# gongweibao/FleetX

Hardware: AMD Instinct MI355X
Metric: tokens/sec (whole node) GPT-3 6.7B hybrid-parallel at 1/2/4/8 MI355X (higher is better)
Workload: dtype bf16; 1 GPU; model=gpt3-6.7B, global_batch=8, seq_len=1024, parallelism=dp1, micro_batch=8, hip_graph=True, grad_reduce_dtype=float32, recompute=False

## Files before the change

### csrc/kernels/bindings.cpp

```cpp
#include <hip/hip_runtime.h>
#include <pybind11/pybind11.h>
#include <pybind11/stl.h>
#include <stdint.h>
#include <string>
#include <stdexcept>
#include <vector>

namespace py = pybind11;
typedef uintptr_t ptr;

#include "fx_api.h"

#define P(x) reinterpret_cast<void*>(x)
#define CP(x) reinterpret_cast<const void*>(x)
#define S(x) reinterpret_cast<hipStream_t>(x)
#define F(x) reinterpret_cast<float*>(x)

static std::vector<long> v3(const std::vector<long>& a) {
  std::vector<long> r(a);
  r.resize(3, 0);
  return r;
}

PYBIND11_MODULE(_kernels, m) {
  m.doc() = "FleetX-AMD HIP kernels (gfx950)";
  m.def("coltile_splits", &fx_coltile_splits);
  m.def("add_ln_fwd", [](int dt, ptr x, ptr bias, ptr res, ptr g, ptr b, ptr s_out, ptr y,
                         ptr mean, ptr rstd, int rows, int h, float eps, float p, uint64_t key,
                         ptr salt, ptr st) {
    fx_add_ln_fwd(dt, CP(x), CP(bias), CP(res), CP(g), CP(b), P(s_out), P(y), F(mean), F(rstd),
                  rows, h, eps, p, key, CP(salt), S(st));
  });
  m.def("ln_bwd_row", [](int dt, ptr dy, ptr s, ptr mean, ptr rstd, ptr g, ptr ds_in, ptr ds_out,
                         ptr dx_out, int rows, int h, float p, uint64_t key, ptr salt, ptr st) {
    fx_ln_bwd_row(dt, CP(dy), CP(s), F(mean), F(rstd), CP(g), CP(ds_in), P(ds_out), P(dx_out),
                  rows, h, p, key, CP(salt), S(st));
  });
  m.def("ln_bwd_cols_blocks", &fx_ln_bwd_cols_blocks);
  m.def("ln_bwd_cols", [](int dt, ptr dy, ptr s, ptr mean, ptr rstd, ptr g, ptr ds_in, ptr ds_out,
                          ptr dx_out, int rows, int h, float p, uint64_t key, ptr part,
                          int with_dbias, ptr fg, ptr tg, int accg, ptr fb, ptr tb, int accb,
                          ptr fx, ptr tx, int accx, ptr salt, ptr st) {
    return fx_ln_bwd_cols(dt, CP(dy), CP(s), F(mean), F(rstd), CP(g), CP(ds_in), P(ds_out),
                          P(dx_out), rows, h, p, key, F(part), with_dbias, F(fg), P(tg), accg,
                          F(fb), P(tb), accb, F(fx), P(tx), accx, CP(salt), S(st));
  }, py::arg("dt"), py::arg("dy"), py::arg("s"), py::arg("mean"), py::arg("rstd"), py::arg("g"),
     py::arg("ds_in"), py::arg("ds_out"), py::arg("dx_out"), py::arg("rows"), py::arg("h"),
     py::arg("p"), py::arg("key"), py::arg("part"), py::arg("with_dbias"), py::arg("fg") = 0,
     py::arg("tg") = 0, py::arg("accg") = 0, py::arg("fb") = 0, py::arg("tb") = 0,
     py::arg("accb") = 0, py::arg("fx") = 0, py::arg("tx") = 0, py::arg("accx") = 0,
     py::arg("salt") = 0, py::arg("st") = 0);
  m.def("coltile_partial", [](int dt, int mode, ptr a, ptr b, ptr mean, ptr rstd, ptr p0, ptr p1,
                              int rows, int cols, int splits, ptr st, ptr cnt, ptr f0, ptr t0,
                              int acc0, ptr f1, ptr t1, int acc1) {
    fx_coltile_partial(dt, mode, CP(a), CP(b), F(mean), F(rstd), F(p0), F(p1), rows, cols, splits,
                       S(st), reinterpret_cast<int*>(cnt), F(f0), P(t0), acc0, F(f1), P(t1),
                       acc1);
  }, py::arg("dt"), py::arg("mode"), py::arg("a"), py::arg("b"), py::arg("mean"), py::arg("rstd"),
     py::arg("p0"), py::arg("p1"), py::arg("rows"), py::arg("cols"), py::arg("splits"),
     py::arg("st"), py::arg("cnt") = 0, py::arg("f0") = 0, py::arg("t0") = 0, py::arg("acc0") = 0,
     py::arg("f1") = 0, py::arg("t1") = 0, py::arg("acc1") = 0);
  m.def("coltile_finalize", [](int dt, ptr part, int splits, int cols, ptr out_f32, ptr out_t,
                               int accumulate, ptr st) {
    fx_coltile_finalize(dt, F(part), splits, cols, F(out_f32), P(out_t), accumulate, S(st));
  });
  m.def("bias_gelu_fwd", [](int dt, int erf, ptr x, ptr bias, ptr y, long n, int cols, ptr st) {
    fx_bias_gelu_fwd(dt, erf, CP(x), CP(bias), P(y), n, cols, S(st));
  });
  m.def("bias_gelu_bwd", [](int dt, int erf, ptr dy, ptr x, ptr bias, ptr dx, ptr part, int rows,
                            int cols, int splits, ptr st, ptr cnt, ptr out_f32, ptr out_t,
                            int acc) {
    fx_bias_gelu_bwd(dt, erf, CP(dy), CP(x), CP(bias), P(dx), F(part), rows, cols, splits, S(st),
                     reinterpret_cast<int*>(cnt), F(out_f32), P(out_t), acc);
  }, py::arg("dt"), py::arg("erf"), py::arg("dy"), py::arg("x"), py::arg("bias"), py::arg("dx"),
     py::arg("part"), py::arg("rows"), py::arg("cols"), py::arg("splits"), py::arg("st"),
     py::arg("cnt") = 0, py::arg("out_f32") = 0, py::arg("out_t") = 0, py::arg("acc") = 0);
  m.def("bias_dropout_add_fwd", [](int dt, ptr x, ptr bias, ptr res, ptr out, long n, int cols,
                                   float p, uint64_t key, ptr salt, ptr st) {
    fx_bias_dropout_add_fwd(dt, CP(x), CP(bias), CP(res), P(out), n, cols, p, key, CP(salt),
                            S(st));
  });
  m.def("dropout_bwd_colsum", [](int dt, ptr dout, ptr dx, ptr part, int rows, int cols,
                                 int splits, float p, uint64_t key, ptr salt, ptr st, ptr cnt,
                                 ptr out_f32, ptr out_t, int acc) {
    fx_dropout_bwd_colsum(dt, CP(dout), P(dx), F(part), rows, cols, splits, p, key, CP(salt), S(st),
                          reinterpret_cast<int*>(cnt), F(out_f32), P(out_t), acc);
  }, py::arg("dt"), py::arg("dout"), py::arg("dx"), py::arg("part"), py::arg("rows"),
     py::arg("cols"), py::arg("splits"), py::arg("p"), py::arg("key"), py::arg("salt"),
     py::arg("st"), py::arg("cnt") = 0, py::arg("out_f32") = 0, py::arg("out_t") = 0,
     py::arg("acc") = 0);
  m.def("dropout_fwd", [](int dt, ptr x, ptr y, long n, float p, uint64_t key, ptr salt,
                          ptr st) {
    fx_dropout_fwd(dt, CP(x), P(y), n, p, key, CP(salt), S(st));
  });
  m.def("ce_stats", [](int dt, ptr logits, ptr labels, int rows, int V, long vstart, ptr mx,
                       ptr sm, ptr tg, int ignore, ptr st) {
    fx_ce_stats(dt, CP(logits), reinterpret_cast<const int64_t*>(labels), rows, V, vstart, F(mx),
                F(sm), F(tg), ignore, S(st));
  });
  m.def("ce_bwd", [](int dt, ptr logits, ptr dx, ptr labels, ptr lse, ptr g, int rows, int V,
                     long vstart, int ignore, ptr st) {
    fx_ce_bwd(dt, CP(logits), P(dx), reinterpret_cast<const int64_t*>(labels), F(lse), F(g), rows,
              V, vstart, ignore, S(st));
  });
  m.def("sumsq_blocks", &fx_sumsq_blocks);
  m.def("sumsq_chunks", [](ptr addr, ptr len, int n, ptr partial, ptr st) {
    fx_sumsq_chunks(reinterpret_cast<const int64_t*>(addr), reinterpret_cast<const int64_t*>(len),
                    n, F(partial), S(st));
  });
  m.def("sumsq_f32", [](ptr x, long n, ptr partial, int blocks, ptr st) {
    fx_sumsq_f32(F(x), n, F(partial), blocks, S(st));
  });
  m.def("sumsq_16", [](int dt, ptr x, long n, ptr partial, int blocks, ptr st) {
    fx_sumsq_16(dt, CP(x), n, F(partial), blocks, S(st));
  });
  m.def("adamw", [](int dt, int flags, ptr p, ptr g, ptr mm, ptr vv, ptr p16, long n, float lr,
                    float b1, float b2, float eps, float wd, float l2, ptr gscale, ptr skip,
                    ptr step, ptr lr_dev, int grid, int nt, int wide, ptr st) {
    return fx_adamw(dt, flags, P(p), CP(g), F(mm), F(vv), P(p16), n, lr, b1, b2, eps, wd, l2,
                    F(gscale), reinterpret_cast<const int*>(skip),
                    reinterpret_cast<const int*>(step), F(lr_dev), grid, nt, wide, S(st));
  });
  m.def("pk_split", [](ptr x, ptr hi, ptr lo, long n, ptr st) {
    fx_pk_split(F(x), P(hi), P(lo), n, S(st));
  });
  m.def("pk_join", [](ptr hi, ptr lo, ptr x, long n, ptr st) {
// ... 177 lines not shown
```

### csrc/kernels/fx_api.h

```cpp
#pragma once
#include <hip/hip_runtime.h>
#include <stdint.h>

extern "C" {
int fx_coltile_splits(int rows, int cols);
void fx_add_ln_fwd(int, const void*, const void*, const void*, const void*, const void*, void*,
                   void*, float*, float*, int, int, float, float, uint64_t, const void*,
                   hipStream_t);
void fx_ln_bwd_row(int, const void*, const void*, const float*, const float*, const void*,
                   const void*, void*, void*, int, int, float, uint64_t, const void*, hipStream_t);
int fx_ln_bwd_cols_blocks(int, int, int);
int fx_ln_bwd_cols(int, const void*, const void*, const float*, const float*, const void*,
                   const void*, void*, void*, int, int, float, uint64_t, float*, int, float*, void*,
                   int, float*, void*, int, float*, void*, int, const void*, hipStream_t);
void fx_coltile_partial(int, int, const void*, const void*, const float*, const float*, float*,
                        float*, int, int, int, hipStream_t, int*, float*, void*, int, float*,
                        void*, int);
void fx_coltile_finalize(int, const float*, int, int, float*, void*, int, hipStream_t);
void fx_bias_gelu_fwd(int, int, const void*, const void*, void*, long, int, hipStream_t);
void fx_bias_gelu_bwd(int, int, const void*, const void*, const void*, void*, float*, int, int, int,
                      hipStream_t, int*, float*, void*, int);
void fx_bias_dropout_add_fwd(int, const void*, const void*, const void*, void*, long, int, float,
                             uint64_t, const void*, hipStream_t);
void fx_dropout_bwd_colsum(int, const void*, void*, float*, int, int, int, float, uint64_t,
                           const void*, hipStream_t, int*, float*, void*, int);
void fx_dropout_fwd(int, const void*, void*, long, float, uint64_t, const void*, hipStream_t);
void fx_ce_stats(int, const void*, const int64_t*, int, int, long, float*, float*, float*, int,
                 hipStream_t);
void fx_ce_bwd(int, const void*, void*, const int64_t*, const float*, const float*, int, int, long,
               int, hipStream_t);
int fx_sumsq_blocks(long n);
void fx_sumsq_f32(const float*, long, float*, int, hipStream_t);
void fx_sumsq_16(int, const void*, long, float*, int, hipStream_t);
void fx_sumsq_chunks(const int64_t*, const int64_t*, int, float*, hipStream_t);
int fx_adamw(int dtype, int flags, void* master, const void* grad, float* m, float* v, void* p16,
             long n, float lr, float beta1, float beta2, float eps, float wd, float l2,
             const float* gscale, const int* skip, const int* step, const float* lr_dev,
             int grid_cap, int nt, int wide, hipStream_t st);
void fx_pk_split(const float*, void*, void*, long, hipStream_t);
void fx_pk_join(const void*, const void*, float*, long, hipStream_t);
void fx_cast_f32(int, const float*, void*, long, hipStream_t);
void fx_accum_f32(int, float*, const void*, long, int, hipStream_t);
void fx_embedding_fwd(int, const int64_t*, const int64_t*, const void*, const void*, void*, int,
                      int, long, long, hipStream_t);
void fx_embedding_bwd(int, const int64_t*, const void*, float*, int, int, long, long,
                      hipStream_t);
void fx_fa_set_dkdv64(int);
void fx_fa_set_dq64(int);
void fx_fa_set_dkdv_vreg(int);
int fx_fa_lab();
int fx_fa_set_stamps(void*);
int fx_flash_fwd(int, const void*, const void*, const void*, void*, float*, const long*, const long*,
                 const long*, const long*, const int*, const float*, long, int, int, int, int, int,
                 int, float, float, uint64_t, const void*, hipStream_t);
int fx_flash_bwd(int, const void*, const void*, const void*, const void*, const void*, const float*,
                 float*, void*, void*, void*, const long*, const long*, const long*, const long*,
                 const long*, const long*, const int*, const float*, long, int, int, int, int, int,
                 int, float, float, uint64_t, const void*, hipStream_t);
int fx_fake_quant_fwd(int, const void*, void*, const float*, int, long, hipStream_t);
void fx_absmax(int, const void*, long, float*, hipStream_t);
int fx_gn_nseg(long, long);
int fx_gn_fwd(int, const void*, const float*, const float*, const float*, const float*, void*,
              double*, float*, float*, int, int, int, long, int, float, int, hipStream_t);
int fx_gn_bwd_reduce(int, const void*, const void*, const float*, const float*, const float*,
                     const float*, const float*, const float*, float*, int, int, int, long, int,
                     int, hipStream_t);
int fx_gn_bwd_apply(int, const void*, const void*, const float*, const float*, const float*,
                    const float*, const float*, const float*, const float*, const float*, void*,
                    int, int, int, long, int, int, hipStream_t);
int fx_transpose16(int, const void*, void*, float*, int, int, long, long, hipStream_t);
int fx_sample(int, const void*, long, int, int, float, int, float, const float*, int64_t*, float*,
              float*, hipStream_t);
int fx_decode_attn(int, const void*, const void*, const void*, void*, const int*, int, int, int,
                   int, int, float*, long, long, long, long, long, long, float, hipStream_t);
int fx_beam_decode_attn(int, const void*, const void*, const void*, const int*, const void*,
                        const void*, const int*, const int*, void*, float*, int, int, int, int, int,
                        int, int, long, long, long, long, long, long, long, long, long, long, float,
                        int, hipStream_t);
void fx_embedding_bwd_sorted(int, const int64_t*, const int64_t*, const void*, float*, int, int,
                             long, long, hipStream_t);
int fx_softmax_fwd(int, int, const void*, const void*, void*, long, int, int, long, float, int,
                   hipStream_t);
int fx_softmax_bwd(int, const void*, const void*, void*, long, int, int, float, int, hipStream_t);
int fx_gemm(int, int, int, int, int, int, int, const void*, long, const void*, long, void*, long,
            const void*, void*, long, int, hipStream_t, float*, float*);
long fx_gemm_ws_bytes(int, int, int, int);
void fx_gemm_set_gm(int);
void fx_gemm_set_geom(int, int);
int fx_gemm_tuned(long*, int);
void fx_gemm_set_tuned(int, int, int, int, int, int, int);
void fx_gemm_set_tune(int);
void fx_gemm_set_persist(int);
void fx_gemm_set_xrect(int);
int fx_decode_gemv(int, int, int, int, int, const void*, long, const void*, long, const void*,
                   const void*, long, void*, long, void*, void*, const long*, int, int, int,
// ... 14 lines not shown
```

### csrc/kernels/norm_eltwise.hip

```cpp
#include "fx_api.h"
#include "fx_common.h"

namespace {

struct DropCfg {
  uint32_t klo, khi, thr;
  float scale;
  int enabled;
  const uint64_t* salt;
};

__device__ __forceinline__ DropCfg resolve_drop(DropCfg d) {
  if (d.enabled && d.salt != nullptr) {
    const uint64_t k = salt_key(((uint64_t)d.khi << 32) | d.klo, *d.salt);
    d.klo = (uint32_t)k;
    d.khi = (uint32_t)(k >> 32);
  }
  return d;
}

__device__ __forceinline__ float drop_apply(float v, uint64_t idx, const DropCfg& d) {
  if (!d.enabled) return v;
  uint32_t h = elem_rand_pair(idx, d.klo, d.khi);
  uint32_t r = (idx & 1) ? (h >> 16) : (h & 0xffffu);
// ... 90 lines not shown
  }
  const float rstd = rsqrtf(wave_sum(var) / h + eps);
#pragma unroll
  for (int i = 0; i < VPT; ++i) {
    const int c = (i * 64 + lane) * 8;
    if (MASK && c >= h) continue;
    float g[8], b[8], o[8];
    load8<T>(gamma + c, g);
    load8<T>(beta + c, b);
#pragma unroll
    for (int j = 0; j < 8; ++j) o[j] = (v[i][j] - mean) * rstd * g[j] + b[j];
    store8<T>(y + base + c, o);
  }
  if (lane == 0) {
    mean_out[row] = mean;
    rstd_out[row] = rstd;
  }
}

template <typename T>
__global__ __launch_bounds__(256) void add_ln_fwd_generic(
    const uint16_t* __restrict__ x, const uint16_t* __restrict__ bias,
    const uint16_t* __restrict__ residual, const uint16_t* __restrict__ gamma,
    const uint16_t* __restrict__ beta, uint16_t* __restrict__ s_out,
    uint16_t* __restrict__ y, float* __restrict__ mean_out, float* __restrict__ rstd_out,
    int rows, int h, float eps, DropCfg drop_) {
  const DropCfg drop = resolve_drop(drop_);
  const int lane = threadIdx.x & 63;
  const int row = blockIdx.x * 4 + (threadIdx.x >> 6);
  if (row >= rows) return;
  const size_t base = (size_t)row * h;
  const int nv = h / 8;
  auto value = [&](int c, float* v) {
    load8<T>(x + base + c, v);
    if (bias) {
      float b[8];
      load8<T>(bias + c, b);
      for (int j = 0; j < 8; ++j) v[j] += b[j];
    }
    if (drop.enabled)
      drop_apply8(v, base + c, drop);
    if (residual) {
      float r[8];
      load8<T>(residual + base + c, r);
      for (int j = 0; j < 8; ++j) v[j] += r[j];
    }
  };
  float sum = 0.f;
  for (int vi = lane; vi < nv; vi += 64) {
    float v[8];
    value(vi * 8, v);
    if (s_out) {
      store8<T>(s_out + base + vi * 8, v);
      for (int j = 0; j < 8; ++j) v[j] = round_to<T>(v[j]);
    }
    for (int j = 0; j < 8; ++j) sum += v[j];
  }
  const float mean = wave_sum(sum) / h;
  float var = 0.f;
  for (int vi = lane; vi < nv; vi += 64) {
    float v[8];
    if (s_out) load8<T>(s_out + base + vi * 8, v); else value(vi * 8, v);
    for (int j = 0; j < 8; ++j) { float d = v[j] - mean; var += d * d; }
  }
  const float rstd = rsqrtf(wave_sum(var) / h + eps);
  for (int vi = lane; vi < nv; vi += 64) {
    float v[8], g[8], b[8], o[8];
    if (s_out) load8<T>(s_out + base + vi * 8, v); else value(vi * 8, v);
    load8<T>(gamma + vi * 8, g);
    load8<T>(beta + vi * 8, b);
    for (int j = 0; j < 8; ++j) o[j] = (v[j] - mean) * rstd * g[j] + b[j];
    store8<T>(y + base + vi * 8, o);
  }
  if (lane == 0) { mean_out[row] = mean; rstd_out[row] = rstd; }
}

template <typename T, int VPT, bool MASK = false>
__global__ __launch_bounds__(256) void ln_bwd_row_kernel(
    const uint16_t* __restrict__ dy, const uint16_t* __restrict__ s,
    const float* __restrict__ mean_in, const float* __restrict__ rstd_in,
    const uint16_t* __restrict__ gamma, const uint16_t* __restrict__ ds_in,
    uint16_t* __restrict__ ds_out, uint16_t* __restrict__ dx_out, int rows, int h,
    DropCfg drop_) {
  const DropCfg drop = resolve_drop(drop_);
  const int lane = threadIdx.x & 63;
  const int row = blockIdx.x * 4 + (threadIdx.x >> 6);
  if (row >= rows) return;
  const size_t base = (size_t)row * h;
  const float mean = mean_in[row], rstd = rstd_in[row];
  float xh[VPT][8], gdy[VPT][8];
  float s1 = 0.f, s2 = 0.f;
#pragma unroll
  for (int i = 0; i < VPT; ++i) {
    const int c = (i * 64 + lane) * 8;
    if (MASK && c >= h) {
#pragma unroll
      for (int j = 0; j < 8; ++j) xh[i][j] = gdy[i][j] = 0.f;
      continue;
    }
    float a[8], g[8], d[8];
    load8<T>(s + base + c, a);
    load8<T>(gamma + c, g);
    load8<T>(dy + base + c, d);
#pragma unroll
    for (int j = 0; j < 8; ++j) {
      xh[i][j] = (a[j] - mean) * rstd;
      gdy[i][j] = d[j] * g[j];
      s1 += gdy[i][j];
      s2 += gdy[i][j] * xh[i][j];
    }
  }
  uint4 dr[VPT];
  if (ds_in) {
#pragma unroll
    for (int i = 0; i < VPT; ++i) {
      const int c = (i * 64 + lane) * 8;
      dr[i] = make_uint4(0, 0, 0, 0);
      if (!MASK || c < h) dr[i] = *reinterpret_cast<const uint4*>(ds_in + base + c);
    }
  }
  const float m1 = wave_sum(s1) / h, m2 = wave_sum(s2) / h;
#pragma unroll
  for (int i = 0; i < VPT; ++i) {
    const int c = (i * 64 + lane) * 8;
    if (MASK && c >= h) continue;
    float o[8];
#pragma unroll
    for (int j = 0; j < 8; ++j) o[j] = rstd * (gdy[i][j] - m1 - xh[i][j] * m2);
    if (ds_in) {
      float r[8];
      unpack8<T>(dr[i], r);
#pragma unroll
      for (int j = 0; j < 8; ++j) o[j] += r[j];
    }
    store8<T>(ds_out + base + c, o);
    if (drop.enabled) {
      drop_apply8(o, base + c, drop);
      store8<T>(dx_out + base + c, o);
    } else if (dx_out != ds_out) {
      store8<T>(dx_out + base + c, o);
    }
  }
}

template <typename T>
__global__ __launch_bounds__(256) void ln_bwd_row_generic(
    const uint16_t* __restrict__ dy, const uint16_t* __restrict__ s,
    const float* __restrict__ mean_in, const float* __restrict__ rstd_in,
    const uint16_t* __restrict__ gamma, const uint16_t* __restrict__ ds_in,
    uint16_t* __restrict__ ds_out, uint16_t* __restrict__ dx_out, int rows, int h,
    DropCfg drop_) {
  const DropCfg drop = resolve_drop(drop_);
  const int lane = threadIdx.x & 63;
  const int row = blockIdx.x * 4 + (threadIdx.x >> 6);
  if (row >= rows) return;
  const size_t base = (size_t)row * h;
  const float mean = mean_in[row], rstd = rstd_in[row];
  const int nv = h / 8;
  float s1 = 0.f, s2 = 0.f;
  for (int vi = lane; vi < nv; vi += 64) {
    float a[8], g[8], d[8];
    load8<T>(s + base + vi * 8, a);
    load8<T>(gamma + vi * 8, g);
    load8<T>(dy + base + vi * 8, d);
    for (int j = 0; j < 8; ++j) {
      float xh = (a[j] - mean) * rstd, gd = d[j] * g[j];
      s1 += gd;
      s2 += gd * xh;
    }
  }
  const float m1 = wave_sum(s1) / h, m2 = wave_sum(s2) / h;
  for (int vi = lane; vi < nv; vi += 64) {
    const int c = vi * 8;
    float a[8], g[8], d[8], o[8];
    load8<T>(s + base + c, a);
    load8<T>(gamma + c, g);
    load8<T>(dy + base + c, d);
    for (int j = 0; j < 8; ++j) o[j] = rstd * (d[j] * g[j] - m1 - (a[j] - mean) * rstd * m2);
    if (ds_in) {
      float r[8];
      load8<T>(ds_in + base + c, r);
      for (int j = 0; j < 8; ++j) o[j] += r[j];
    }
    store8<T>(ds_out + base + c, o);
    if (drop.enabled) {
      drop_apply8(o, base + c, drop);
      store8<T>(dx_out + base + c, o);
    } else if (dx_out != ds_out) {
      store8<T>(dx_out + base + c, o);
    }
  }
}

template <typename T, int VPT, int WPR, bool MASK, bool DB>
__global__ __launch_bounds__(256, 2) void ln_bwd_cols_kernel(
    const uint16_t* __restrict__ dy, const uint16_t* __restrict__ s,
    const float* __restrict__ mean_in, const float* __restrict__ rstd_in,
    const uint16_t* __restrict__ gamma, const uint16_t* __restrict__ ds_in,
    uint16_t* __restrict__ ds_out, uint16_t* __restrict__ dx_out, int rows, int h,
    int rows_per_group, float* __restrict__ part, DropCfg drop_) {
  constexpr int NG = 4 / WPR;
  __shared__ float red[4 * 512 * VPT];
  __shared__ float xs[2][4][2];
  const DropCfg drop = resolve_drop(drop_);
  const int lane = threadIdx.x & 63, w = threadIdx.x >> 6;
  const int grp = w / WPR, half = w % WPR;
  const int hw = h / WPR, cbase = half * hw;
  const int r0 = min(rows, (blockIdx.x * NG + grp) * rows_per_group);
  const int r1 = min(rows, r0 + rows_per_group);
  uint4 gp[VPT];
  float ag[VPT][8], ab[VPT][8], ax[DB ? VPT : 1][8];
// ... 77 lines not shown
      unpack8<T>(ca[i], a);
      unpack8<T>(cd[i], d);
      unpack8<T>(gp[i], g);
#pragma unroll
      for (int j = 0; j < 8; ++j) o[j] = rstd * (d[j] * g[j] - m1 - (a[j] - mean) * rstd * m2);
      if (ds_in) {
        float rr[8];
        unpack8<T>(cr[i], rr);
#pragma unroll
        for (int j = 0; j < 8; ++j) o[j] += rr[j];
      }
      store8<T>(ds_out + base + c, o);
      if (drop.enabled) {
        drop_apply8(o, base + c, drop);
        store8<T>(dx_out + base + c, o);
      } else if (dx_out != ds_out) {
        store8<T>(dx_out + base + c, o);
      }
      if (DB) {
#pragma unroll
        for (int j = 0; j < 8; ++j) ax[i][j] += round_to<T>(o[j]);
      }
    }
  }
#pragma unroll
  for (int arr = 0; arr < (DB ? 3 : 2); ++arr) {
    __syncthreads();
#pragma unroll
    for (int i = 0; i < VPT; ++i) {
      const int c = (i * 64 + lane) * 8;
      if (MASK && c >= hw) continue;
#pragma unroll
      for (int j = 0; j < 8; ++j)
        red[grp * h + cbase + c + j] = arr == 0 ? ag[i][j] : arr == 1 ? ab[i][j] : ax[DB ? i : 0][j];
    }
    __syncthreads();
    float* out = part + ((size_t)arr * gridDim.x + blockIdx.x) * h;
    for (int c = threadIdx.x; c < h; c += 256) {
      float v = red[c];
#pragma unroll
      for (int q = 1; q < NG; ++q) v += red[q * h + c];
      out[c] = v;
    }
  }
}

struct LnColsOut {
  float* f32[3];
  uint16_t* t16[3];
  int acc[3];
};
template <typename T>
__global__ __launch_bounds__(256) void ln_cols_finalize_kernel(const float* __restrict__ part,
                                                               int G, int h, LnColsOut f) {
  __shared__ float tr[8][132];
  const int arr = blockIdx.y;
  const float* p = part + (size_t)arr * G * h;
  const int q = threadIdx.x & 31, sr = threadIdx.x >> 5;
  const int c0 = blockIdx.x * 128 + q * 4;
  floatx4 acc = {0.f, 0.f, 0.f, 0.f};
  if (c0 < h) {
    for (int k0 = sr; k0 < G; k0 += 128) {
      floatx4 v[16];
#pragma unroll
      for (int u = 0; u < 16; ++u) {
        const int k = k0 + 8 * u;
        v[u] = k < G ? *reinterpret_cast<const floatx4*>(p + (size_t)k * h + c0)
                     : floatx4{0.f, 0.f, 0.f, 0.f};
      }
#pragma unroll
      for (int u = 0; u < 16; ++u) acc += v[u];
    }
  }
#pragma unroll
  for (int j = 0; j < 4; ++j) tr[sr][q * 4 + j] = acc[j];
  __syncthreads();
  const int c = threadIdx.x, gc = blockIdx.x * 128 + c;
  if (c >= 128 || gc >= h) return;
  float sum = 0.f;
#pragma unroll
  for (int t = 0; t < 8; ++t) sum += tr[t][c];
  if (f.f32[arr]) f.f32[arr][gc] = f.acc[arr] ? f.f32[arr][gc] + sum : sum;
  if (f.t16[arr]) f.t16[arr][gc] = Elt<T>::from_f(sum);
}

typedef __attribute__((address_space(1))) float gf32;
typedef __attribute__((address_space(1))) int gi32;

__device__ __forceinline__ void st_part(float* p, float v) {
  __hip_atomic_store((gf32*)p, v, __ATOMIC_RELAXED, __HIP_MEMORY_SCOPE_AGENT);
}

struct ColFin {
  int* cnt;
  float* f32[2];
  uint16_t* t16[2];
  int acc[2];
};

template <typename T>
__device__ __forceinline__ void colsum_tail(const float* __restrict__ p0,
                                            const float* __restrict__ p1, int cols, int np,
                                            const ColFin& f) {
  __shared__ int last;
  asm volatile("s_waitcnt vmcnt(0)" ::: "memory");
  __syncthreads();
  if (threadIdx.x == 0) {
    const int t = __hip_atomic_fetch_add((gi32*)(f.cnt + 32 * blockIdx.x), 1, __ATOMIC_RELAXED,
                                         __HIP_MEMORY_SCOPE_AGENT);
    last = t == (int)gridDim.y - 1;
    if (last)
      __hip_atomic_store((gi32*)(f.cnt + 32 * blockIdx.x), 0, __ATOMIC_RELAXED,
                         __HIP_MEMORY_SCOPE_AGENT);
  }
  __syncthreads();
  if (!last) return;
  __builtin_amdgcn_fence(__ATOMIC_ACQUIRE, "wavefront");
  __shared__ float tr[8][132];
  const int q = threadIdx.x & 31, sr = threadIdx.x >> 5;
  const int c0 = blockIdx.x * 128 + q * 4;
  const int splits = gridDim.y;
  for (int which = 0; which < np; ++which) {
    const float* p = which ? p1 : p0;
    floatx4 s = {0.f, 0.f, 0.f, 0.f};
    if (c0 < cols) {
      const auto rs = __builtin_amdgcn_make_buffer_rsrc(const_cast<float*>(p), 0,
                                                        splits * cols * 4, 0x00020000);
      for (int k0 = sr; k0 < splits; k0 += 128) {
        floatx4 v[16];
#pragma unroll
        for (int u = 0; u < 16; ++u) {
          const int k = k0 + 8 * u;
          const uint32_t off = k < splits ? (uint32_t)(k * cols + c0) * 4u : 0x80000000u;
          v[u] = __builtin_bit_cast(floatx4, __builtin_amdgcn_raw_buffer_load_b128(rs, off, 0, 16));
        }
#pragma unroll
        for (int u = 0; u < 16; ++u) s += v[u];
      }
    }
#pragma unroll
    for (int j = 0; j < 4; ++j) tr[sr][q * 4 + j] = s[j];
    __syncthreads();
    const int c = threadIdx.x, gc = blockIdx.x * 128 + c;
    if (c < 128 && gc < cols) {
      float sum = 0.f;
#pragma unroll
      for (int t = 0; t < 8; ++t) sum += tr[t][c];
      if (f.f32[which]) f.f32[which][gc] = f.acc[which] ? f.f32[which][gc] + sum : sum;
      if (f.t16[which]) f.t16[which][gc] = Elt<T>::from_f(sum);
    }
    __syncthreads();
  }
}

template <typename T, int MODE>
__global__ __launch_bounds__(256) void coltile_partial_kernel(
    const uint16_t* __restrict__ a, const uint16_t* __restrict__ b,
    const float* __restrict__ mean, const float* __restrict__ rstd,
    float* __restrict__ p0, float* __restrict__ p1, int rows, int cols, int rows_per_split,
    ColFin fin) {
  __shared__ float red[2][16][129];
  const int tx = threadIdx.x & 15, ty = threadIdx.x >> 4;
  const int col = blockIdx.x * 128 + tx * 8;
  const int r0 = blockIdx.y * rows_per_split;
  const int r1 = min(rows, r0 + rows_per_split);
  float acc0[8], acc1[8];
// ... 376 lines not shown
      LNB_CASE(8)
      default:
        FX_DISPATCH_T(dtype, ln_bwd_row_generic<T><<<grid, block, 0, st>>>(
                                 DY, S, mean, rstd, G, DI, DS, DX, rows, h, d));
    }
  } else if (h % 8 == 0 && h < 8 * 512) {
#define LNBM_CASE(V)                                                                      \
  case V:                                                                                 \
    FX_DISPATCH_T(dtype, ln_bwd_row_kernel<T, V, true><<<grid, block, 0, st>>>(           \
                             DY, S, mean, rstd, G, DI, DS, DX, rows, h, d));              \
    break;
    switch ((h + 511) / 512) {
      LNBM_CASE(1) LNBM_CASE(2) LNBM_CASE(3) LNBM_CASE(4) LNBM_CASE(5) LNBM_CASE(6)
      LNBM_CASE(7) LNBM_CASE(8)
    }
#undef LNBM_CASE
  } else {
    FX_DISPATCH_T(dtype, ln_bwd_row_generic<T><<<grid, block, 0, st>>>(
                             DY, S, mean, rstd, G, DI, DS, DX, rows, h, d));
  }
#undef LNB_CASE
}

static int ln_cols_wpr(int h) { return h <= 1536 ? 1 : h <= 3072 ? 2 : 4; }
static int ln_cols_rows_per_group(int rows, int h) {
  const int ng = 4 / ln_cols_wpr(h);
  int rpg = (rows + 512 * ng - 1) / (512 * ng);
  return rpg < 2 ? 2 : rpg;
}
extern "C" int fx_ln_bwd_cols_blocks(int rows, int h, int max_h) {
  if (rows <= 0 || h > (max_h < 4096 ? max_h : 4096) || h % (8 * ln_cols_wpr(h))) return 0;
  const int ng = 4 / ln_cols_wpr(h), rpg = ln_cols_rows_per_group(rows, h);
  return (rows + ng * rpg - 1) / (ng * rpg);
}

extern "C" int fx_ln_bwd_cols(int dtype, const void* dy, const void* s, const float* mean,
                              const float* rstd, const void* gamma, const void* ds_in,
                              void* ds_out, void* dx_out, int rows, int h, float p, uint64_t key,
                              float* part, int with_dbias, float* fg, void* tg, int accg,
                              float* fb, void* tb, int accb, float* fx, void* tx, int accx,
                              const void* salt, hipStream_t st) {
  const int G = fx_ln_bwd_cols_blocks(rows, h, 4096);
  if (G == 0) return -1;
  const int wpr = ln_cols_wpr(h), hw = h / wpr;
  const int rpg = ln_cols_rows_per_group(rows, h);
  DropCfg d = make_drop(p, key, salt);
  auto DY = (const uint16_t*)dy;
  auto S = (const uint16_t*)s;
  auto GM = (const uint16_t*)gamma;
  auto DI = (const uint16_t*)ds_in;
  auto DS = (uint16_t*)ds_out;
  auto DX = (uint16_t*)dx_out;
  const int vpt = (hw + 511) / 512;
  const bool mask = hw % 512 != 0;
#define LNC_GO(V, W, M, DB)                                                                   \
  FX_DISPATCH_T(dtype, ln_bwd_cols_kernel<T, V, W, M, DB><<<G, 256, 0, st>>>(                 \
                           DY, S, mean, rstd, GM, DI, DS, DX, rows, h, rpg, part, d))
#define LNC_M(V, W)                                                                           \
  if (mask) {                                                                                 \
    if (with_dbias) { LNC_GO(V, W, true, true); } else { LNC_GO(V, W, true, false); }         \
  } else {                                                                                    \
    if (with_dbias) { LNC_GO(V, W, false, true); } else { LNC_GO(V, W, false, false); }       \
  }
#define LNC_V(V)                                                                              \
  case V:                                                                                     \
    if (wpr == 1) { LNC_M(V, 1) } else if (wpr == 2) { LNC_M(V, 2) } else { LNC_M(V, 4) }     \
    break;
  switch (vpt) {
    LNC_V(1) LNC_V(2) LNC_V(3)
    default: return -1;
  }
#undef LNC_V
#undef LNC_M
#undef LNC_GO
  LnColsOut f;
  f.f32[0] = fg; f.f32[1] = fb; f.f32[2] = fx;
  f.t16[0] = (uint16_t*)tg; f.t16[1] = (uint16_t*)tb; f.t16[2] = (uint16_t*)tx;
  f.acc[0] = accg; f.acc[1] = accb; f.acc[2] = accx;
  dim3 grid((h + 127) / 128, with_dbias ? 3 : 2);
  FX_DISPATCH_T(dtype, ln_cols_finalize_kernel<T><<<grid, 256, 0, st>>>(part, G, h, f));
  return 0;
}

extern "C" void fx_coltile_partial(int dtype, int mode, const void* a, const void* b,
                                   const float* mean, const float* rstd, float* p0, float* p1,
                                   int rows, int cols, int splits, hipStream_t st, int* cnt,
                                   float* f0, void* t0, int acc0, float* f1, void* t1, int acc1) {
  const ColFin fin = make_fin(cnt, f0, t0, acc0, f1, t1, acc1);
  int rps = (rows + splits - 1) / splits;
  dim3 grid((cols + 127) / 128, splits), block(256);
  auto A = (const uint16_t*)a;
  auto B = (const uint16_t*)b;
  if (mode == 0) {
    FX_DISPATCH_T(dtype, coltile_partial_kernel<T, 0><<<grid, block, 0, st>>>(
                             A, B, mean, rstd, p0, p1, rows, cols, rps, fin));
  } else {
    FX_DISPATCH_T(dtype, coltile_partial_kernel<T, 1><<<grid, block, 0, st>>>(
                             A, B, mean, rstd, p0, p1, rows, cols, rps, fin));
  }
}

extern "C" void fx_coltile_finalize(int dtype, const float* part, int splits, int cols,
                                    float* out_f32, void* out_t, int accumulate, hipStream_t st) {
  dim3 grid((cols + 255) / 256), block(256);
  FX_DISPATCH_T(dtype, coltile_finalize_kernel<T><<<grid, block, 0, st>>>(
                           part, splits, cols, out_f32, (uint16_t*)out_t, accumulate));
}

extern "C" void fx_bias_gelu_fwd(int dtype, int erf, const void* x, const void* bias, void* y,
                                 long n, int cols, hipStream_t st) {
  long n8 = n / 8;
  if (erf) {
    FX_DISPATCH_T(dtype, bias_gelu_fwd_kernel<T, true><<<grid_for(n8), 256, 0, st>>>(
                             (const uint16_t*)x, (const uint16_t*)bias, (uint16_t*)y, n8, cols));
  } else {
    FX_DISPATCH_T(dtype, bias_gelu_fwd_kernel<T, false><<<grid_for(n8), 256, 0, st>>>(
                             (const uint16_t*)x, (const uint16_t*)bias, (uint16_t*)y, n8, cols));
  }
}

extern "C" void fx_bias_gelu_bwd(int dtype, int erf, const void* dy, const void* x,
                                 const void* bias, void* dx, float* part, int rows, int cols,
                                 int splits, hipStream_t st, int* cnt, float* out_f32,
                                 void* out_t, int acc) {
  const ColFin fin = make_fin(cnt, out_f32, out_t, acc, nullptr, nullptr, 0);
  int rps = (rows + splits - 1) / splits;
  dim3 grid((cols + 127) / 128, splits), block(256);
  if (erf) {
    FX_DISPATCH_T(dtype, bias_gelu_bwd_kernel<T, true><<<grid, block, 0, st>>>(
                             (const uint16_t*)dy, (const uint16_t*)x, (const uint16_t*)bias,
                             (uint16_t*)dx, part, rows, cols, rps, fin));
  } else {
    FX_DISPATCH_T(dtype, bias_gelu_bwd_kernel<T, false><<<grid, block, 0, st>>>(
                             (const uint16_t*)dy, (const uint16_t*)x, (const uint16_t*)bias,
                             (uint16_t*)dx, part, rows, cols, rps, fin));
  }
}

extern "C" void fx_bias_dropout_add_fwd(int dtype, const void* x, const void* bias,
                                        const void* residual, void* out, long n, int cols, float p,
                                        uint64_t key, const void* salt, hipStream_t st) {
  DropCfg d = make_drop(p, key, salt);
  long n8 = n / 8;
  FX_DISPATCH_T(dtype, bias_dropout_add_fwd_kernel<T><<<grid_for(n8), 256, 0, st>>>(
                           (const uint16_t*)x, (const uint16_t*)bias, (const uint16_t*)residual,
                           (uint16_t*)out, n8, cols, d));
}

extern "C" void fx_dropout_bwd_colsum(int dtype, const void* dout, void* dx, float* part,
                                      int rows, int cols, int splits, float p, uint64_t key,
                                      const void* salt, hipStream_t st, int* cnt,
                                      float* out_f32, void* out_t, int acc) {
  const ColFin fin = make_fin(cnt, out_f32, out_t, acc, nullptr, nullptr, 0);
  DropCfg d = make_drop(p, key, salt);
  int rps = (rows + splits - 1) / splits;
  dim3 grid((cols + 127) / 128, splits), block(256);
  FX_DISPATCH_T(dtype, dropout_bwd_colsum_kernel<T><<<grid, block, 0, st>>>(
                           (const uint16_t*)dout, (uint16_t*)dx, part, rows, cols, rps, d, fin));
}

extern "C" void fx_dropout_fwd(int dtype, const void* x, void* y, long n, float p, uint64_t key,
                               const void* salt, hipStream_t st) {
  DropCfg d = make_drop(p, key, salt);
  long n8 = n / 8;
  FX_DISPATCH_T(dtype, dropout_fwd_kernel<T><<<grid_for(n8), 256, 0, st>>>(
                           (const uint16_t*)x, (uint16_t*)y, n, d));
// ... 2 lines not shown
```

### fleetx_amd/ops/norm.py

```python
import os

import torch

from . import _lib
from ..parallel import grad_sink as sink, rng as _rng


_TICKETS = {}


def colsum_tickets(device, cols):
    st = torch.cuda.current_stream(device).cuda_stream
    need = 32 * ((cols + 127) // 128)
    t = _TICKETS.get(st)
    if t is None or t.numel() < need:
        t = torch.zeros(max(4096, need), dtype=torch.int32, device=device)
        _TICKETS[st] = t
    return t.data_ptr()


_TARGET_KW = (("f0", "t0", "acc0"), ("f1", "t1", "acc1"))


def _coltile(mode, x, aux, rows, cols, targets):
    k = _lib.kernels()
    splits = k.coltile_splits(rows, cols)
    p0 = torch.empty(splits, cols, device=x.device, dtype=torch.float32)
    p1 = torch.empty_like(p0) if mode == 0 else None
    fin = {}
    for (kf, kt, ka), (f32, t16, acc) in zip(_TARGET_KW, targets):
        if f32:
            fin[kf], fin[ka] = f32, acc
        else:
            fin[kt] = t16
    k.coltile_partial(_lib.dt_code(x.dtype), mode, x.data_ptr(), *aux, p0.data_ptr(),
                      _lib.ptr(p1), rows, cols, splits, _lib.stream(),
                      cnt=colsum_tickets(x.device, cols), **fin)


def _col_target(prm, direct, cols, like):
    if direct:
        mg, acc = sink.open_write(prm)
        return (mg.data_ptr(), 0, int(acc)), None
    g = torch.empty(cols, device=like.device, dtype=like.dtype)
    return (0, g.data_ptr(), 0), g


def col_sum(x, cols):
    if not _lib.vec8_ok(cols, x):
        return x.reshape(-1, cols).float().sum(0).to(x.dtype)
    out = torch.empty(cols, device=x.device, dtype=x.dtype)
    _coltile(1, x, (0, 0, 0), x.numel() // cols, cols, [(0, out.data_ptr(), 0)])
    return out


def col_sum_f32(x, dst, accumulate=False):
    cols = dst.numel()
    x = x.contiguous()
    if not _lib.vec8_ok(cols, x):
        sink.store_or_add(dst, x.reshape(-1, cols).float().sum(0).view_as(dst), accumulate)
        return dst
    if dst.dtype != torch.float32 or not dst.is_contiguous():
        raise ValueError("col_sum_f32: dst must be contiguous fp32")
    _coltile(1, x, (0, 0, 0), x.numel() // cols, cols, [(dst.data_ptr(), 0, int(accumulate))])
    return dst


def _dropout_ref(x, p, key):
    if p <= 0.0:
        return x
    m = _rng.keep_mask(x.shape, p, key, x.device)
    return torch.where(m, x * (1.0 / (1.0 - p)), torch.zeros_like(x))


def _ln_bwd_cols_max_h():
    mode = os.environ.get("FLEETX_LN_BWD_FUSED", "1")
    return {"0": 0, "2": 4096}.get(mode, 1536)


def _ln_bwd_cols(k, dc, dy, s, mean, rstd, weight, ctx, ds_in, ds, dx, rows, h):
    G = k.ln_bwd_cols_blocks(rows, h, 4096)
    with_db = bool(ctx.has_bias)
    part = torch.empty(3 if with_db else 2, G, h, device=dy.device, dtype=torch.float32)
    prms = (weight, ctx.lnbias, ctx.bias if with_db else None)
    outs, grads = [], []
    for prm in prms:
        t, g = ((0, 0, 0), None) if prm is None else \
            _col_target(prm, sink.fused(prm, fp32_contiguous=True), h, dy)
        outs.append(t)
        grads.append(g)
    (fg, tg, ag), (fb, tb, ab), (fx, tx, ax) = outs
    rc = k.ln_bwd_cols(dc, dy.data_ptr(), s.data_ptr(), mean.data_ptr(), rstd.data_ptr(),
                       weight.data_ptr(), _lib.ptr(ds_in), ds.data_ptr(), dx.data_ptr(), rows, h,
                       float(ctx.p), ctx.key, part.data_ptr(), int(with_db), fg, tg, ag, fb, tb,
                       ab, fx, tx, ax, _rng.device_salt_ptr(), _lib.stream())
    if rc != 0:
        raise RuntimeError("ln_bwd_cols: shape rows=%d h=%d not covered" % (rows, h))
    for prm, (f32, _, _) in zip(prms, outs):
        if f32:
            sink.close_write(prm)
    return grads


class _AddLayerNorm(torch.autograd.Function):
    @staticmethod
    def forward(ctx, x, bias, residual, weight, lnbias, eps, p, key, store_sum):
        h = x.shape[-1]
        rows = x.numel() // h
        ctx.p, ctx.key, ctx.has_bias, ctx.has_res = p, key, bias is not None, residual is not None
        ctx.h = h
        x = x.contiguous()
        if _lib.vec8_ok(h, x, bias, residual, weight, lnbias):
            k = _lib.kernels()
            fused = bias is not None or residual is not None or p > 0
            s = torch.empty_like(x) if fused else None
            y = torch.empty_like(x)
            mean = torch.empty(rows, device=x.device, dtype=torch.float32)
            rstd = torch.empty_like(mean)
            k.add_ln_fwd(_lib.dt_code(x.dtype), x.data_ptr(), _lib.ptr(bias), _lib.ptr(residual),
                         weight.data_ptr(), lnbias.data_ptr(), _lib.ptr(s), y.data_ptr(),
                         mean.data_ptr(), rstd.data_ptr(), rows, h, float(eps), float(p), key,
                         _rng.device_salt_ptr(), _lib.stream())
            s_saved = s if s is not None else x
            if s is None and store_sum:
                s = x
        else:
            v = x
            if bias is not None or residual is not None or p > 0:
                v = x.float() if bias is None else x.float() + bias.float()
                v = _dropout_ref(v, p, key)
                if residual is not None:
                    v = v + residual.float()
                v = v.to(x.dtype)
            s_saved = v
            s = v if (store_sum or bias is not None or residual is not None or p > 0) else None
            vf = v.float()
            mean = vf.mean(-1).reshape(-1)
            var = ((vf - mean.view(*vf.shape[:-1], 1)) ** 2).mean(-1).reshape(-1)
            rstd = torch.rsqrt(var + eps)
            y = ((vf - mean.view(*vf.shape[:-1], 1)) * rstd.view(*vf.shape[:-1], 1) * weight.float()
                 + lnbias.float()).to(x.dtype)
        ctx.save_for_backward(s_saved, mean, rstd, weight)
        ctx.lnbias, ctx.bias = lnbias, bias
        ctx.return_sum = s is not None
        if s is None:
            return y
        return s, y

    @staticmethod
    def backward(ctx, *grads):
        if ctx.return_sum:
            ds_in, dy = grads
        else:
            ds_in, dy = None, grads[0]
        s, mean, rstd, weight = ctx.saved_tensors
        h = ctx.h
        rows = s.numel() // h
        dy = dy.contiguous()
        if ds_in is not None:
            ds_in = ds_in.contiguous()
        if _lib.vec8_ok(h, dy, ds_in, s, weight):
            k = _lib.kernels()
            dc = _lib.dt_code(dy.dtype)
            ds = torch.empty_like(dy)
            dx = torch.empty_like(dy) if ctx.p > 0 else ds
            if k.ln_bwd_cols_blocks(rows, h, _ln_bwd_cols_max_h()) > 0:
                dw, db, dbias = _ln_bwd_cols(k, dc, dy, s, mean, rstd, weight, ctx, ds_in, ds, dx,
                                             rows, h)
                dres = ds if ctx.has_res else None
                return dx, dbias, dres, dw, db, None, None, None, None
            k.ln_bwd_row(dc, dy.data_ptr(), s.data_ptr(), mean.data_ptr(), rstd.data_ptr(),
                         weight.data_ptr(), _lib.ptr(ds_in), ds.data_ptr(), dx.data_ptr(), rows, h,
                         float(ctx.p), ctx.key, _rng.device_salt_ptr(), _lib.stream())
            direct = sink.fused(weight) and sink.fused(ctx.lnbias)
            (tw, dw), (tb, db) = (_col_target(prm, direct, h, dy) for prm in (weight, ctx.lnbias))
            _coltile(0, dy, (s.data_ptr(), mean.data_ptr(), rstd.data_ptr()), rows, h, [tw, tb])
            if direct:
                sink.close_write(weight)
                sink.close_write(ctx.lnbias)
            dbias = None
            if ctx.has_bias:
                if sink.fused(ctx.bias):
                    mg, acc = sink.open_write(ctx.bias)
                    col_sum_f32(dx, mg, acc)
                    sink.close_write(ctx.bias)
                else:
                    dbias = col_sum(dx, h)
        else:
            sf = s.float().reshape(rows, h)
            xh = (sf - mean.view(rows, 1)) * rstd.view(rows, 1)
            g = dy.float().reshape(rows, h) * weight.float()
            m1 = g.mean(-1, keepdim=True)
            m2 = (g * xh).mean(-1, keepdim=True)
            dsf = rstd.view(rows, 1) * (g - m1 - xh * m2)
            if ds_in is not None:
                dsf = dsf + ds_in.float().reshape(rows, h)
            ds = dsf.to(dy.dtype).reshape(dy.shape)
            dx = _dropout_ref(ds, ctx.p, ctx.key)
            dw = sink.deliver(weight, (dy.float().reshape(rows, h) * xh).sum(0), weight.dtype,
                              on_gpu=True)
            db = sink.deliver(ctx.lnbias, dy.float().reshape(rows, h).sum(0), weight.dtype,
                              on_gpu=True)
            dbias = None
            if ctx.has_bias:
                dbias = sink.deliver(ctx.bias, dx.float().reshape(rows, h).sum(0), dy.dtype,
                                     on_gpu=True)
        dres = ds if ctx.has_res else None
        return dx, dbias, dres, dw, db, None, None, None, None


def add_layer_norm(x, bias, residual, weight, lnbias, eps=1e-5, p=0.0, key=0):
    return _AddLayerNorm.apply(x, bias, residual, weight, lnbias, eps, p, key, True)


def layer_norm(x, weight, bias, eps=1e-5):
    return _AddLayerNorm.apply(x, None, None, weight, bias, eps, 0.0, 0, False)


def layer_norm_keep_input(x, weight, bias, eps=1e-5):
    return _AddLayerNorm.apply(x, None, None, weight, bias, eps, 0.0, 0, True)


class FusedLayerNorm(torch.nn.Module):

    def __init__(self, hidden, eps=1e-5, dtype=None, device=None):
        super().__init__()
        self.weight = torch.nn.Parameter(torch.ones(hidden, dtype=dtype, device=device))
        self.bias = torch.nn.Parameter(torch.zeros(hidden, dtype=dtype, device=device))
        self.weight._fx_fused_wgrad_ok = True
        self.bias._fx_fused_wgrad_ok = True
        self.eps = eps
        self.normalized_shape = (hidden,)

    def forward(self, x):
        return layer_norm(x, self.weight, self.bias, self.eps)
```

Measured before the change: 28650 tokens/s.

## Add persistent slab LayerNorm backward kernel with LDS column-gradient accumulation

Adds a persistent LayerNorm backward kernel for hidden sizes 2048-4096. Each wavefront walks rows in a grid-stride loop, double-buffers the next row's loads, and accumulates the gamma, beta and optional bias column gradients into per-wave fp32 slabs in LDS. The block reduces those slabs into one partial row per block, so the finalize kernel sums only about one partial per CU instead of many. It is enabled by default through an environment flag and costs large dynamic shared memory per block, which limits occupancy. It also disables fp contraction in the row kernel for numerical consistency.

```diff
diff --git a/csrc/kernels/bindings.cpp b/csrc/kernels/bindings.cpp
--- a/csrc/kernels/bindings.cpp
+++ b/csrc/kernels/bindings.cpp
@@ -42,6 +42,20 @@
                           int with_dbias, ptr fg, ptr tg, int accg, ptr fb, ptr tb, int accb,
                           ptr fx, ptr tx, int accx, ptr salt, ptr st) {
     return fx_ln_bwd_cols(dt, CP(dy), CP(s), F(mean), F(rstd), CP(g), CP(ds_in), P(ds_out),
+                          P(dx_out), rows, h, p, key, F(part), with_dbias, F(fg), P(tg), accg,
+                          F(fb), P(tb), accb, F(fx), P(tx), accx, CP(salt), S(st));
+  }, py::arg("dt"), py::arg("dy"), py::arg("s"), py::arg("mean"), py::arg("rstd"), py::arg("g"),
+     py::arg("ds_in"), py::arg("ds_out"), py::arg("dx_out"), py::arg("rows"), py::arg("h"),
+     py::arg("p"), py::arg("key"), py::arg("part"), py::arg("with_dbias"), py::arg("fg") = 0,
+     py::arg("tg") = 0, py::arg("accg") = 0, py::arg("fb") = 0, py::arg("tb") = 0,
+     py::arg("accb") = 0, py::arg("fx") = 0, py::arg("tx") = 0, py::arg("accx") = 0,
+     py::arg("salt") = 0, py::arg("st") = 0);
+  m.def("ln_bwd_slab_blocks", &fx_ln_bwd_slab_blocks);
+  m.def("ln_bwd_slab", [](int dt, ptr dy, ptr s, ptr mean, ptr rstd, ptr g, ptr ds_in, ptr ds_out,
+                          ptr dx_out, int rows, int h, float p, uint64_t key, ptr part,
+                          int with_dbias, ptr fg, ptr tg, int accg, ptr fb, ptr tb, int accb,
+                          ptr fx, ptr tx, int accx, ptr salt, ptr st) {
+    return fx_ln_bwd_slab(dt, CP(dy), CP(s), F(mean), F(rstd), CP(g), CP(ds_in), P(ds_out),
                           P(dx_out), rows, h, p, key, F(part), with_dbias, F(fg), P(tg), accg,
                           F(fb), P(tb), accb, F(fx), P(tx), accx, CP(salt), S(st));
   }, py::arg("dt"), py::arg("dy"), py::arg("s"), py::arg("mean"), py::arg("rstd"), py::arg("g"),
diff --git a/csrc/kernels/fx_api.h b/csrc/kernels/fx_api.h
--- a/csrc/kernels/fx_api.h
+++ b/csrc/kernels/fx_api.h
@@ -11,6 +11,10 @@
                    const void*, void*, void*, int, int, float, uint64_t, const void*, hipStream_t);
 int fx_ln_bwd_cols_blocks(int, int, int);
 int fx_ln_bwd_cols(int, const void*, const void*, const float*, const float*, const void*,
+                   const void*, void*, void*, int, int, float, uint64_t, float*, int, float*, void*,
+                   int, float*, void*, int, float*, void*, int, const void*, hipStream_t);
+int fx_ln_bwd_slab_blocks(int, int, int);
+int fx_ln_bwd_slab(int, const void*, const void*, const float*, const float*, const void*,
                    const void*, void*, void*, int, int, float, uint64_t, float*, int, float*, void*,
                    int, float*, void*, int, float*, void*, int, const void*, hipStream_t);
 void fx_coltile_partial(int, int, const void*, const void*, const float*, const float*, float*,
diff --git a/csrc/kernels/norm_eltwise.hip b/csrc/kernels/norm_eltwise.hip
--- a/csrc/kernels/norm_eltwise.hip
+++ b/csrc/kernels/norm_eltwise.hip
@@ -196,6 +196,7 @@
     const uint16_t* __restrict__ gamma, const uint16_t* __restrict__ ds_in,
     uint16_t* __restrict__ ds_out, uint16_t* __restrict__ dx_out, int rows, int h,
     DropCfg drop_) {
+#pragma clang fp contract(off)
   const DropCfg drop = resolve_drop(drop_);
   const int lane = threadIdx.x & 63;
   const int row = blockIdx.x * 4 + (threadIdx.x >> 6);
@@ -240,7 +241,7 @@
     if (MASK && c >= h) continue;
     float o[8];
 #pragma unroll
-    for (int j = 0; j < 8; ++j) o[j] = rstd * (gdy[i][j] - m1 - xh[i][j] * m2);
+    for (int j = 0; j < 8; ++j) o[j] = rstd * __builtin_fmaf(-m2, xh[i][j], gdy[i][j] - m1);
     if (ds_in) {
       float r[8];
       unpack8<T>(dr[i], r);
@@ -484,6 +485,159 @@
   for (int t = 0; t < 8; ++t) sum += tr[t][c];
   if (f.f32[arr]) f.f32[arr][gc] = f.acc[arr] ? f.f32[arr][gc] + sum : sum;
   if (f.t16[arr]) f.t16[arr][gc] = Elt<T>::from_f(sum);
+}
+
+template <int VPT>
+struct LnSlabRow {
+  uint4 a[VPT], d[VPT], r[VPT];
+  float mean, rstd;
+};
+
+template <int VPT, bool DI>
+__device__ __forceinline__ void ln_slab_request(LnSlabRow<VPT>& R, const uint16_t* dy,
+                                                const uint16_t* s,
+                                                const uint16_t* ds_in,
+                                                const float* __restrict__ mean_in,
+                                                const float* __restrict__ rstd_in, int row, int h,
+                                                int lane) {
+  const size_t base = (size_t)row * h;
+#pragma unroll
+  for (int i = 0; i < VPT; ++i)
+    R.a[i] = *reinterpret_cast<const uint4*>(s + base + (i * 64 + lane) * 8);
+#pragma unroll
+  for (int i = 0; i < VPT; ++i)
+    R.d[i] = *reinterpret_cast<const uint4*>(dy + base + (i * 64 + lane) * 8);
+  if (DI) {
+#pragma unroll
+    for (int i = 0; i < VPT; ++i)
+      R.r[i] = *reinterpret_cast<const uint4*>(ds_in + base + (i * 64 + lane) * 8);
+  }
+  R.mean = mean_in[row];
+  R.rstd = rstd_in[row];
+}
+
+template <typename T, int VPT, bool DB, bool DI, bool DROP>
+__device__ __forceinline__ void ln_slab_row(const LnSlabRow<VPT>& R, const uint4* gl, float* slab,
+                                            uint16_t* ds_out,
+                                            uint16_t* dx_out, int row, int h, int lane,
+                                            const DropCfg& drop) {
+#pragma clang fp contract(off)
+  const size_t base = (size_t)row * h;
+  const float mean = R.mean, rstd = R.rstd;
+  DropCfg dc = drop;
+  dc.enabled = DROP;
+  floatx4* sl = reinterpret_cast<floatx4*>(slab);
+  float s1 = 0.f, s2 = 0.f;
+#pragma unroll
+  for (int i = 0; i < VPT; ++i) {
+    float a[8], g[8], d[8], xh[8];
+    unpack8<T>(R.a[i], a);
+    unpack8<T>(gl[i * 64 + lane], g);
+    unpack8<T>(R.d[i], d);
+#pragma unroll
+    for (int j = 0; j < 8; ++j) {
+      xh[j] = (a[j] - mean) * rstd;
+      const float gdy = d[j] * g[j];
+      s1 += gdy;
+      s2 += gdy * xh[j];
+    }
+#pragma unroll
+    for (int hf = 0; hf < 2; ++hf) {
+      floatx4& pg = sl[((0 * VPT + i) * 2 + hf) * 64 + lane];
+      floatx4& pb = sl[((1 * VPT + i) * 2 + hf) * 64 + lane];
+      floatx4 vg = pg, vb = pb;
+#pragma unroll
+      for (int j = 0; j < 4; ++j) {
+        vg[j] = __builtin_fmaf(d[4 * hf + j], xh[4 * hf + j], vg[j]);
+        vb[j] += d[4 * hf + j];
+      }
+      pg = vg;
+      pb = vb;
+    }
+  }
+  const float m1 = wave_sum(s1) / h, m2 = wave_sum(s2) / h;
+#pragma unroll
+  for (int i = 0; i < VPT; ++i) {
+    const int c = (i * 64 + lane) * 8;
+    float a[8], g[8], d[8], o[8];
+    unpack8<T>(R.a[i], a);
+    unpack8<T>(gl[i * 64 + lane], g);
+    unpack8<T>(R.d[i], d);
+#pragma unroll
+    for (int j = 0; j < 8; ++j)
+      o[j] = rstd * __builtin_fmaf(-m2, (a[j] - mean) * rstd, d[j] * g[j] - m1);
+    if (DI) {
+      float r[8];
+      unpack8<T>(R.r[i], r);
+#pragma unroll
+      for (int j = 0; j < 8; ++j) o[j] += r[j];
+    }
+    store8<T>(ds_out + base + c, o);
+    if (DROP) {
+      drop_apply8(o, base + c, dc);
+      store8<T>(dx_out + base + c, o);
+    } else if (dx_out != ds_out) {
+      store8<T>(dx_out + base + c, o);
+    }
+    if (DB) {
+#pragma unroll
+      for (int hf = 0; hf < 2; ++hf) {
+        floatx4& px = sl[((2 * VPT + i) * 2 + hf) * 64 + lane];
+        floatx4 vx = px;
+#pragma unroll
+        for (int j = 0; j < 4; ++j) vx[j] += round_to<T>(o[4 * hf + j]);
+        px = vx;
+      }
+    }
+  }
+}
+
+template <typename T, int VPT, bool DB, bool DI, bool DROP>
+__global__ __launch_bounds__(256) void ln_bwd_slab_kernel(
+    const uint16_t* dy, const uint16_t* s, const float* __restrict__ mean_in,
+    const float* __restrict__ rstd_in, const uint16_t* gamma, const uint16_t* ds_in,
+    uint16_t* ds_out, uint16_t* dx_out, int rows, int h, float* __restrict__ part,
+    DropCfg drop_) {
+  extern __shared__ __attribute__((aligned(16))) float slabs[];
+  constexpr int NS = DB ? 3 : 2;
+  constexpr int NQ = NS * VPT * 128;
+  const DropCfg drop = resolve_drop(drop_);
+  const int lane = threadIdx.x & 63, W = blockDim.x >> 6;
+  const int w = __builtin_amdgcn_readfirstlane(threadIdx.x >> 6);
+  float* slab = slabs + (size_t)w * NQ * 4;
+  for (int q = lane; q < NQ; q += 64)
+    reinterpret_cast<floatx4*>(slab)[q] = floatx4{0.f, 0.f, 0.f, 0.f};
+  uint4* gl = reinterpret_cast<uint4*>(slabs + (size_t)W * NQ * 4);
+  for (int q = threadIdx.x; q < VPT * 64; q += blockDim.x)
+    gl[q] = reinterpret_cast<const uint4*>(gamma)[q];
+  __syncthreads();
+  const int nw = gridDim.x * W, last = rows - 1;
+  int r = blockIdx.x * W + w;
+  LnSlabRow<VPT> A, B;
+  if (r < rows) {
+    ln_slab_request<VPT, DI>(A, dy, s, ds_in, mean_in, rstd_in, r, h, lane);
+    for (;;) {
+      ln_slab_request<VPT, DI>(B, dy, s, ds_in, mean_in, rstd_in, min(r + nw, last), h, lane);
+      __builtin_amdgcn_sched_barrier(0);
+      ln_slab_row<T, VPT, DB, DI, DROP>(A, gl, slab, ds_out, dx_out, r, h, lane, drop);
+      r += nw;
+      if (r >= rows) break;
+      ln_slab_request<VPT, DI>(A, dy, s, ds_in, mean_in, rstd_in, min(r + nw, last), h, lane);
+      __builtin_amdgcn_sched_barrier(0);
+      ln_slab_row<T, VPT, DB, DI, DROP>(B, gl, slab, ds_out, dx_out, r, h, lane, drop);
+      r += nw;
+      if (r >= rows) break;
+    }
+  }
+  __syncthreads();
+  const floatx4* sl = reinterpret_cast<const floatx4*>(slabs);
+  for (int q = threadIdx.x; q < NQ; q += blockDim.x) {
+    floatx4 v = sl[q];
+    for (int k = 1; k < W; ++k) v += sl[k * NQ + q];
+    const int arr = q / (VPT * 128), rem = q % (VPT * 128);
+    const int col = ((rem >> 7) * 64 + (rem & 63)) * 8 + ((rem >> 6) & 1) * 4;
+    *reinterpret_cast<floatx4*>(part + ((size_t)arr * gridDim.x + blockIdx.x) * h + col) = v;
+  }
 }
 
 typedef __attribute__((address_space(1))) float gf32;
@@ -1026,6 +1180,77 @@
   return 0;
 }
 
+static int ln_slab_cus() {
+  static int n = 0;
+  if (n == 0) {
+    int dev = 0;
+    hipDeviceProp_t pr;
+    n = (hipGetDevice(&dev) == hipSuccess && hipGetDeviceProperties(&pr, dev) == hipSuccess &&
+         pr.multiProcessorCount > 0) ? pr.multiProcessorCount : 256;
+  }
+  return n;
+}
+static int ln_slab_waves(int h, int with_dbias) {
+  const int fit = (160 * 1024 - h * 2) / ((with_dbias ? 3 : 2) * h * 4);
+  return fit < 4 ? fit : 4;
+}
+extern "C" int fx_ln_bwd_slab_blocks(int rows, int h, int with_dbias) {
+  if (rows <= 0 || h < 2048 || h > 4096 || h % 512) return 0;
+  const int W = ln_slab_waves(h, with_dbias), cus = ln_slab_cus();
+  const int need = (rows + W - 1) / W;
+  return need < cus ? need : cus;
+}
+
+extern "C" int fx_ln_bwd_slab(int dtype, const void* dy, const void* s, const float* mean,
+                              const float* rstd, const void* gamma, const void* ds_in,
+                              void* ds_out, void* dx_out, int rows, int h, float p, uint64_t key,
+                              float* part, int with_dbias, float* fg, void* tg, int accg,
+                              float* fb, void* tb, int accb, float* fx, void* tx, int accx,
+                              const void* salt, hipStream_t st) {
+  const int G = fx_ln_bwd_slab_blocks(rows, h, with_dbias);
+  if (G == 0) return -1;
+  const int W = ln_slab_waves(h, with_dbias);
+  const size_t smem = (size_t)W * (with_dbias ? 3 : 2) * h * sizeof(float) + (size_t)h * 2;
+  const DropCfg d = make_drop(p, key, salt);
+  auto DY = (const uint16_t*)dy;
+  auto S = (const uint16_t*)s;
+  auto GM = (const uint16_t*)gamma;
+  auto DI = (const uint16_t*)ds_in;
+  auto DS = (uint16_t*)ds_out;
+  auto DX = (uint16_t*)dx_out;
+#define LNS_GO(V, DB, HAS_DI, DROP)                                                             \
+  FX_DISPATCH_T(dtype, {                                                                        \
+    auto kern = ln_bwd_slab_kernel<T, V, DB, HAS_DI, DROP>;                                     \
+    if (smem > 65536)                                                                           \
+      (void)hipFuncSetAttribute((const void*)kern, hipFuncAttributeMaxDynamicSharedMemorySize,  \
+                                (int)smem);                                                     \
+    kern<<<G, 64 * W, smem, st>>>(DY, S, mean, rstd, GM, DI, DS, DX, rows, h, part, d);         \
+  })
+#define LNS_DROP(V, DB, HAS_DI)                                                                 \
+  if (d.enabled) { LNS_GO(V, DB, HAS_DI, true); } else { LNS_GO(V, DB, HAS_DI, false); }
+#define LNS_DI(V, DB)                                                                           \
+  if (DI) { LNS_DROP(V, DB, true) } else { LNS_DROP(V, DB, false) }
+#define LNS_V(V)                                                                                \
+  case V:                                                                                       \
+    if (with_dbias) { LNS_DI(V, true) } else { LNS_DI(V, false) }                               \
+    break;
+  switch (h / 512) {
+    LNS_V(4) LNS_V(5) LNS_V(6) LNS_V(7) LNS_V(8)
+    default: return -1;
+  }
+#undef LNS_V
+#undef LNS_DI
+#undef LNS_DROP
+#undef LNS_GO
+  LnColsOut f;
+  f.f32[0] = fg; f.f32[1] = fb; f.f32[2] = fx;
+  f.t16[0] = (uint16_t*)tg; f.t16[1] = (uint16_t*)tb; f.t16[2] = (uint16_t*)tx;
+  f.acc[0] = accg; f.acc[1] = accb; f.acc[2] = accx;
+  dim3 grid((h + 127) / 128, with_dbias ? 3 : 2);
+  FX_DISPATCH_T(dtype, ln_cols_finalize_kernel<T><<<grid, 256, 0, st>>>(part, G, h, f));
+  return 0;
+}
+
 extern "C" void fx_coltile_partial(int dtype, int mode, const void* a, const void* b,
                                    const float* mean, const float* rstd, float* p0, float* p1,
                                    int rows, int cols, int splits, hipStream_t st, int* cnt,
diff --git a/fleetx_amd/ops/norm.py b/fleetx_amd/ops/norm.py
--- a/fleetx_amd/ops/norm.py
+++ b/fleetx_amd/ops/norm.py
@@ -78,9 +78,14 @@
     return {"0": 0, "2": 4096}.get(mode, 1536)
 
 
-def _ln_bwd_cols(k, dc, dy, s, mean, rstd, weight, ctx, ds_in, ds, dx, rows, h):
-    G = k.ln_bwd_cols_blocks(rows, h, 4096)
+def _ln_bwd_slab_on():
+    return (os.environ.get("FLEETX_LN_BWD_SLAB", "1") != "0"
+            and os.environ.get("FLEETX_LN_BWD_FUSED", "1") == "1")
+
+
+def _ln_bwd_cols(k, dc, dy, s, mean, rstd, weight, ctx, ds_in, ds, dx, rows, h, slab=False):
     with_db = bool(ctx.has_bias)
+    G = k.ln_bwd_slab_blocks(rows, h, int(with_db)) if slab else k.ln_bwd_cols_blocks(rows, h, 4096)
     part = torch.empty(3 if with_db else 2, G, h, device=dy.device, dtype=torch.float32)
     prms = (weight, ctx.lnbias, ctx.bias if with_db else None)
     outs, grads = [], []
@@ -90,12 +95,14 @@
         outs.append(t)
         grads.append(g)
     (fg, tg, ag), (fb, tb, ab), (fx, tx, ax) = outs
-    rc = k.ln_bwd_cols(dc, dy.data_ptr(), s.data_ptr(), mean.data_ptr(), rstd.data_ptr(),
-                       weight.data_ptr(), _lib.ptr(ds_in), ds.data_ptr(), dx.data_ptr(), rows, h,
-                       float(ctx.p), ctx.key, part.data_ptr(), int(with_db), fg, tg, ag, fb, tb,
-                       ab, fx, tx, ax, _rng.device_salt_ptr(), _lib.stream())
+    launch = k.ln_bwd_slab if slab else k.ln_bwd_cols
+    rc = launch(dc, dy.data_ptr(), s.data_ptr(), mean.data_ptr(), rstd.data_ptr(),
+                weight.data_ptr(), _lib.ptr(ds_in), ds.data_ptr(), dx.data_ptr(), rows, h,
+                float(ctx.p), ctx.key, part.data_ptr(), int(with_db), fg, tg, ag, fb, tb,
+                ab, fx, tx, ax, _rng.device_salt_ptr(), _lib.stream())
     if rc != 0:
-        raise RuntimeError("ln_bwd_cols: shape rows=%d h=%d not covered" % (rows, h))
+        raise RuntimeError("ln_bwd_%s: shape rows=%d h=%d not covered"
+                           % ("slab" if slab else "cols", rows, h))
     for prm, (f32, _, _) in zip(prms, outs):
         if f32:
             sink.close_write(prm)
@@ -164,9 +171,10 @@
             dc = _lib.dt_code(dy.dtype)
             ds = torch.empty_like(dy)
             dx = torch.empty_like(dy) if ctx.p > 0 else ds
-            if k.ln_bwd_cols_blocks(rows, h, _ln_bwd_cols_max_h()) > 0:
+            slab = _ln_bwd_slab_on() and k.ln_bwd_slab_blocks(rows, h, int(ctx.has_bias)) > 0
+            if slab or k.ln_bwd_cols_blocks(rows, h, _ln_bwd_cols_max_h()) > 0:
                 dw, db, dbias = _ln_bwd_cols(k, dc, dy, s, mean, rstd, weight, ctx, ds_in, ds, dx,
-                                             rows, h)
+                                             rows, h, slab)
                 dres = ds if ctx.has_res else None
                 return dx, dbias, dres, dw, db, None, None, None, None
             k.ln_bwd_row(dc, dy.data_ptr(), s.data_ptr(), mean.data_ptr(), rstd.data_ptr(),
```

After: 28740 tokens/s (median of 6 runs). Within noise of the previous version (+0.3%).
